# jchristopherson/nonlin

Hardware: AMD Instinct MI355X
Metric: LM iterations/sec on m=4096,n=256 fp64; FD-Jacobian GB/s vs HBM peak (higher is better)
Workload: dtype f64

## Files before the change

nonlin_amd/csrc/nlh_common.h:

```cpp
#pragma once
#include <hip/hip_runtime.h>
#include <stdint.h>
#include <type_traits>

#define NLH_WAVE 64

enum NlhStage : int32_t {
    ST_NEED_JAC = 0,
    ST_HAVE_JAC = 1,
    ST_NE_READY = 2,
    ST_NEED_QR = 3,
    ST_QR_READY = 4,
    ST_TRIAL_READY = 5,
    ST_TRIAL_DONE = 6,
    ST_DONE = 7,
    ST_NEED_PCHOL = 8
};

struct LmState {
    double fnorm, fnorm1, par, delta, xnorm, gnorm, pnorm;
    double temp1n;
    double tailsq;
    int32_t iter, neval, njac;
    int32_t stage;
// ... 394 lines not shown
            for (int h = 0; h < 2; ++h) {
                const double av = a[u + h];
                const bool gt = av > prev;
                const double t = (gt ? prev : av) / (gt ? av : prev), tsq = t * t;
                const double d = (prev == 0.0) ? 0.0 : tsq;
                if (gt && prev != 0.0 && tsq != 1.0) newmax |= 1u << (u + h);
                dd[h] = d;
                prev = fmax(prev, av);
            }
            ddst[u >> 1] = make_double2(dd[0], dd[1]);
        }
        tflags[tid] = (int)newmax;
        __syncthreads();
        if (wid == cw) {
            const int nl = (cl + EL - 1) / EL;
            double d[EL];
            const double2 *mine = reinterpret_cast<const double2 *>(dsv + lane * (EL + 2));
#pragma unroll
            for (int u = 0; u < EL / 2; ++u) { const double2 v2 = mine[u]; d[2 * u] = v2.x; d[2 * u + 1] = v2.y; }
            unsigned long long nm = 0;
#pragma unroll
            for (int k = 0; k < TPR; ++k) nm |= (unsigned long long)(unsigned)tflags[lane * TPR + k] << (k * E);
            const unsigned long long mask = __ballot(nm == 0);
            double t = carry[1];
            const int ntrip = (nl + 7) >> 3;
#pragma unroll 1
            for (int g = 0; g < ntrip; ++g) {
                const unsigned m8 = (unsigned)(mask >> (8 * g)) & 0xffu;
                if (m8 == 0xffu) {
#pragma unroll
                    for (int q = 0; q < 8; ++q) {
                        t = nlh_wave_shr1(t);
#pragma unroll
                        for (int u = 0; u < EL; ++u) t = t + d[u];
                    }
                } else {
#pragma unroll 1
                    for (int q = 0; q < 8; ++q) {
                        t = nlh_wave_shr1(t);
                        if ((m8 >> q) & 1u) {
#pragma unroll
                            for (int u = 0; u < EL; ++u) t = t + d[u];
                        } else if (REGGEN) {
#pragma unroll
                            for (int u = 0; u < EL; ++u) {
                                t = t * (((nm >> u) & 1ull) ? d[u] : 1.0);
                                t = t + d[u];
                            }
                        } else {
                            const int l = 8 * g + q;
                            const unsigned long long nml = ((unsigned long long)(unsigned)__builtin_amdgcn_readlane((int)(nm >> 32), l) << 32)
                                                           | (unsigned)__builtin_amdgcn_readlane((int)nm, l);
#pragma unroll
                            for (int qd = 0; qd < EL; qd += 16) {
                                if (((nml >> qd) & 0xffffull) == 0) {
#pragma unroll
                                    for (int u = qd; u < qd + 16; ++u) t = t + d[u];
                                } else {
#pragma unroll
                                    for (int u = qd; u < qd + 16; ++u) {
                                        t = t * (((nml >> u) & 1ull) ? d[u] : 1.0);
                                        t = t + d[u];
                                    }
                                }
                            }
                        }
                    }
                }
            }
            const int lo = __builtin_amdgcn_readlane(__double2loint(t), 8 * ntrip - 1);
            const int hi = __builtin_amdgcn_readlane(__double2hiint(t), 8 * ntrip - 1);
            double mx = mx_in;
#pragma unroll
            for (int w = 0; w < nw; ++w) mx = fmax(mx, wmax[w]);
            if (lane == 0) { carry[1] = __hiloint2double(hi, lo); carry[0] = mx; }
        }
    }
    __syncthreads();
    const double r = carry[0] * sqrt(1.0 + carry[1]);
    __syncthreads();
    return r;
}

__device__ __forceinline__ void nlh_lds_barrier() { asm volatile("s_waitcnt lgkmcnt(0)\n\ts_barrier" ::: "memory"); }

__device__ __forceinline__ bool nlh_odd_ulps(double c, double inv2ulp)
{
    const double z = c * inv2ulp;
    return z != floor(z);
}
template <int EL>
__device__ __forceinline__ double ordered_possum_wave_int(const double (&d)[EL], double s0, bool &ok)
{
    const long long sb = __double_as_longlong(s0);
    const long long es = sb >> 52;
    const double ulp = __longlong_as_double((es - 52) << 52), hu = 0.5 * ulp, inv2ulp = 0.5 / ulp;
    const double C = __longlong_as_double((es << 52) | (1ll << 51)), lim = 0.25 * __longlong_as_double(es << 52);
    double c0 = 0.0, c1 = 0.0;
    bool fine = true;
#pragma unroll
    for (int u = 0; u < EL; ++u) {
        const double x = d[u];
        fine = fine && (x <= lim);
        const double t = C + x, q = t - C, r = x - q;
        const bool tie = fabs(r) == hu;
        if (__builtin_expect(__builtin_amdgcn_ballot_w64(tie) != 0ull, 0)) {
            const double f = x - hu;
            const double a0 = tie ? f + (nlh_odd_ulps(c0 + f, inv2ulp) ? ulp : 0.0) : q;
            const double a1 = tie ? f + (nlh_odd_ulps(c1 + f, inv2ulp) ? 0.0 : ulp) : q;
            c0 = c0 + a0;
            c1 = c1 + a1;
        } else {
            c0 = c0 + q;
            c1 = c1 + q;
        }
    }
#pragma unroll
    for (int off = 1; off < 64; off <<= 1) {
        const double r0 = __shfl_down(c0, off, 64), r1 = __shfl_down(c1, off, 64);
        const double n0 = c0 + (nlh_odd_ulps(c0, inv2ulp) ? r1 : r0);
        const double n1 = c1 + (nlh_odd_ulps(c1, inv2ulp) ? r0 : r1);
        c0 = n0; c1 = n1;
    }
    const double totl = (sb & 1ll) ? c1 : c0;
    const double tot = __hiloint2double(__builtin_amdgcn_readfirstlane(__double2hiint(totl)), __builtin_amdgcn_readfirstlane(__double2loint(totl)));
    const double out = s0 + tot;
    ok = (__builtin_amdgcn_ballot_w64(!fine) == 0ull) && ((__double_as_longlong(out) >> 52) == es);
    return out;
}

template <int EL, int BSZ, typename Get>
__device__ double norm2_flang_block_lanes_pipe(Get get, int len, double *cd, double *aux, double *wm)
{
    constexpr int CAP = 64 * EL, PADCAP = CAP + 128, E = CAP / BSZ, TPR = EL / E, nw = BSZ / 64;
    static_assert(CAP % BSZ == 0 && EL % E == 0 && E % 2 == 0, "chunk must split evenly");
    const int tid = threadIdx.x, lane = tid & 63, wid = tid >> 6;
    const bool prep = wid < nw, chain = (wid == nw);
    const int nch = (len + CAP - 1) / CAP, i0 = tid * E;
    int *tflags = reinterpret_cast<int *>(aux + 8);
    auto loadabs = [&](int c, double (&a)[E]) __attribute__((always_inline)) {
        const int base = c * CAP, cl = min(CAP, len - base);
#pragma unroll
        for (int u = 0; u < E; ++u) a[u] = (i0 + u < cl) ? fabs(get(base + i0 + u)) : 0.0;
    };
    auto scanmax = [&](int c, const double (&a)[E]) __attribute__((always_inline)) {
        double lm = 0.0;
#pragma unroll
        for (int u = 0; u < E; ++u) lm = fmax(lm, a[u]);
        double sc = lm;
#pragma unroll
        for (int off = 1; off < 64; off <<= 1) {
            const double o = __shfl_up(sc, off, 64);
            if (lane >= off) sc = fmax(sc, o);
        }
        double ex = __shfl_up(sc, 1, 64);
        if (lane == 0) ex = 0.0;
        if (lane == 63) wm[c * nw + wid] = sc;
        return ex;
    };
    double a0[E], a1[E], ex0 = 0.0;
    __syncthreads();
    if (prep) {
        loadabs(0, a0);
        if (nch > 1) loadabs(1, a1);
        ex0 = scanmax(0, a0);
    }
// ... 288 lines not shown
```

nonlin_amd/csrc/nlh_qrx.hip:

```cpp
#include "nlh_qrx.h"
#include "nlh_common.h"
#include "../../include/nonlin_hip.h"
#include <type_traits>
#include <cstdio>
#include <cstdlib>
#include <algorithm>

#ifndef QRX_C
#define QRX_C 10
#endif
#define QRX_TR 64
#define QRX_PAD_ROWS 160
#ifndef QRX_AUX_LOAD
#define QRX_AUX_LOAD 0
#endif
#ifndef QRX_AUX_STORE
#define QRX_AUX_STORE 1
#endif
#ifndef QRX_UF
#define QRX_UF(flush) 16
#endif

typedef unsigned int qrx_u32x2 __attribute__((ext_vector_type(2)));
typedef unsigned int qrx_u32x4 __attribute__((ext_vector_type(4)));
// ... 105 lines not shown

__global__ void __launch_bounds__(256)
k_qrx_init_norms(int m, int n, int ld, int coff, size_t tst, const double *__restrict__ T, QrxWs w, LmVecs v,
                 const LmState *__restrict__ st)
{
    __shared__ __attribute__((aligned(16))) double cd[64 * 64 + 128];
    __shared__ __attribute__((aligned(16))) double aux[40 + 128];
    const int p = w.plist ? w.plist[blockIdx.y] : (int)blockIdx.y, k = blockIdx.x;
    if (p < 0 || (st && st[p].stage != ST_NEED_QR)) return;
    const double *a = T + (size_t)p * tst;
    const double nr = norm2_flang_block_lanes<64, 256>([&](int i) { return a[qrx_at(i, coff + k, ld)]; }, m, cd, aux);
    if (threadIdx.x == 0) {
        v.acnorm[(size_t)p * n + k] = nr;
        w.rdiag[(size_t)p * n + k] = nr;
        w.wa[(size_t)p * n + k] = nr;
        v.ipvt[(size_t)p * n + k] = k;
    }
}

template <bool NORMS>
__global__ void __launch_bounds__(256)
k_qrx_init(int m, int n, int ld, int coff, size_t tst, double *__restrict__ T, const double *__restrict__ fall, QrxWs w, LmVecs v,
           const LmState *__restrict__ st)
{
    const int p = blockIdx.x;
    if (st && st[p].stage != ST_NEED_QR) return;
    const int tid = threadIdx.x, BS = blockDim.x;
    double *a = T + (size_t)p * tst;
    const double *f = fall + (size_t)p * m;
    for (int i = tid; i < m; i += BS) a[qrx_at(i, coff + n, ld)] = f[i];
    for (int k = tid; NORMS && k < n; k += BS) {
        double mx = 0.0, sq = 0.0;
        auto step = [&](double vv) {
            const double av = fabs(vv);
            if (mx == 0.0) {
                mx = av;
            } else if (av > mx) {
                const double t = mx / av, tsq = t * t;
                sq = sq * tsq;
                sq = sq + tsq;
                mx = av;
            } else if (av != 0.0) {
                const double t = av / mx;
                sq = sq + t * t;
            }
        };
        const int nblk = (m + 7) >> 3;
        const double *colp = a + (size_t)(coff + k) * 8;
        double xa[8], xb[8];
        auto ld8 = [&](double (&x)[8], int b) {
#pragma unroll
            for (int r = 0; r < 8; ++r) x[r] = colp[(size_t)b * ld * 8 + r];
        };
        ld8(xa, 0);
        for (int b = 0; b < nblk; b += 2) {
            if (b + 1 < nblk) ld8(xb, b + 1);
#pragma unroll
            for (int r = 0; r < 8; ++r) if (b * 8 + r < m) step(xa[r]);
            if (b + 2 < nblk) ld8(xa, b + 2);
            if (b + 1 < nblk) {
#pragma unroll
                for (int r = 0; r < 8; ++r) if ((b + 1) * 8 + r < m) step(xb[r]);
            }
        }
        const double nr = mx * sqrt(1.0 + sq);
        v.acnorm[(size_t)p * n + k] = nr;
        w.rdiag[(size_t)p * n + k] = nr;
        w.wa[(size_t)p * n + k] = nr;
        v.ipvt[(size_t)p * n + k] = k;
    }
    for (int k = tid; k <= n; k += BS) w.src[(size_t)p * (n + 1) + k] = coff + k;
    for (int c = tid; c < ld; c += BS) w.slotof[(size_t)p * ld + c] = c >= coff ? c - coff : -1;
}

#define QRX_LONG_EL 48
#define QRX_LONG_THREADS 256
#ifndef QRX_LONG_GU
#define QRX_LONG_GU 8
#endif
#ifndef QRX_LONG_SU
#define QRX_LONG_SU 4
#endif
#ifndef QRX_PIV64_WG
#define QRX_PIV64_WG 1
#endif
#define QRX_LONG_MAXCH 96
template <int QRX_NL, bool LONG = false, bool FEW = false>
__global__ void __launch_bounds__(LONG ? QRX_LONG_THREADS : 256, (QRX_NL == 32 && !FEW) ? 4 : (QRX_NL == 64 && !FEW && !LONG) ? QRX_PIV64_WG : 1)
k_qrx_pivot(int p0, int m, int n, int ld, int coff, size_t tst, size_t vst, int j, int cur, int np, int flush, double *__restrict__ T, QrxWs w,
            double *__restrict__ Rall, LmVecs v, const LmState *__restrict__ st)
{
    __shared__ __attribute__((aligned(16))) double cd[LONG ? 2 * (64 * QRX_LONG_EL + 128) : (64 * QRX_NL + (FEW ? 256 : 128))];
    __shared__ __attribute__((aligned(16))) double aux[LONG ? 8 + 256 : 40 + 128];
    __shared__ double wmx[LONG ? 3 * QRX_LONG_MAXCH : 1];
    __shared__ double red[64];
    const int p = p0 + blockIdx.x;
    if (st && st[p].stage != ST_NEED_QR) return;
    const int tid = threadIdx.x, BS = blockDim.x, ldp = n + 1;
#ifdef QRX_DBG_CLK
    long long clk[6]; clk[0] = wall_clock64();
#endif
    int *redi = reinterpret_cast<int *>(red + 32);
    double *rdiag = w.rdiag + (size_t)p * n, *wa = w.wa + (size_t)p * n;
    int32_t *src = w.src + (size_t)p * ldp;
    int32_t *ipvt = v.ipvt + (size_t)p * n;
    double *tpc = w.tp + ((size_t)p * 2 + cur) * QRX_C * ldp;
    double *R = Rall + (size_t)p * n * n;

    const bool onecand = (n - j <= BS);
    int32_t *slotof = w.slotof + (size_t)p * ld;
    const bool fresh = (flush & 2) != 0;
    if (fresh) {
        for (int c = tid; c < ld; c += BS) slotof[c] = (c - coff >= j && c - coff <= n) ? c - coff : -1;
        for (int k = j + tid; k <= n; k += BS) src[k] = coff + k;
    }
    double bv = 0.0, my_tk[QRX_C - 1];
    int bk = 0x7fffffff, my_src = 0, my_ipvt = 0;
    if (onecand) {
        const int k = j + tid;
        if (k < n) {
            bv = rdiag[k]; bk = k;
            my_src = fresh ? coff + k : src[k]; my_ipvt = ipvt[k];
#pragma unroll
            for (int q = 0; q < QRX_C - 1; ++q) my_tk[q] = (q < np) ? tpc[(size_t)q * ldp + k] : 0.0;
        }
    } else {
        for (int k = j + tid; k < n; k += BS) {
            const double d = rdiag[k];
            if (bk == 0x7fffffff || d > bv) { bv = d; bk = k; }
        }
    }
    double rd_j = 0.0, wa_j = 0.0;
    int src_j = 0, ipvt_j = 0, src_0 = 0;
    if (tid == 0) { rd_j = rdiag[j]; wa_j = wa[j]; src_j = fresh ? coff + j : src[j]; ipvt_j = ipvt[j]; src_0 = src[0]; }
    __shared__ uint32_t amx[3 * 16];
    const int kmax = (QRX_NL == 32 && onecand) ? j + block_argmax_first_norms(bv, bk != 0x7fffffff, amx) : block_argmax_first(bv, bk, red, redi);
    double *pub = red + 40;
    int *pubi = reinterpret_cast<int *>(pub + QRX_C);
    if (onecand) {
        if (j + tid == kmax) {
#pragma unroll
            for (int q = 0; q < QRX_C - 1; ++q) pub[q] = my_tk[q];
            pubi[0] = my_src; pubi[1] = my_ipvt;
        }
    } else if (tid == 0) {
        pubi[0] = fresh ? coff + kmax : src[kmax]; pubi[1] = ipvt[kmax];
    } else if (tid <= np) {
        pub[tid - 1] = tpc[(size_t)(tid - 1) * ldp + kmax];
    }
    __syncthreads();
    const int srck = pubi[0];
#ifdef QRX_DBG_CLK
    clk[1] = wall_clock64();
#endif
    double tk[QRX_C];
#pragma unroll
    for (int q = 0; q < QRX_C; ++q) tk[q] = (q < QRX_C - 1 && q < np) ? pub[q] : 0.0;
    if (kmax != j) {
        if (tid == 0) {
            rdiag[kmax] = rd_j;
            wa[kmax] = wa_j;
            ipvt[j] = pubi[1]; ipvt[kmax] = ipvt_j;
            if (j == 0) {
                slotof[src_0] = -1;
                slotof[srck] = kmax;
            } else {
                src[kmax] = src_j;
                slotof[src_j] = kmax;
                slotof[srck] = -1;
            }
        }
        if (tid < np) tpc[(size_t)tid * ldp + kmax] = tpc[(size_t)tid * ldp + j];
        for (int i = tid; i < j; i += BS) {
            const double t = R[(size_t)j * n + i];
            R[(size_t)j * n + i] = R[(size_t)kmax * n + i];
            R[(size_t)kmax * n + i] = t;
        }
    } else if (tid == 0) {
        slotof[srck] = -1;
    }
    const bool move0 = (j == 0 && kmax != 0);
    if (LONG && (flush & 8)) {
        if (tid == 0) {
            QrxStep s;
            s.ajnorm = 0.0; s.ajj = 0.0; s.kmax = kmax; s.srck = srck; s.t0 = np ? tk[0] : 0.0;
            w.step[p] = s;
        }
        return;
    }
    const int src0 = coff;
    const double *__restrict__ Vc = w.V + ((size_t)p * 2 + cur) * QRX_C * vst;
    double *__restrict__ Vn = (flush & 1) ? w.V + ((size_t)p * 2 + (cur ^ 1)) * QRX_C * vst
                                    : w.V + (((size_t)p * 2 + cur) * QRX_C + np) * vst;
    double *Tp = T + (size_t)p * tst;
    const bool staged = !LONG && (m - j <= 64 * QRX_NL);
    double *stage = cd;
    auto spos = [](int i) __attribute__((always_inline)) { return FEW ? i + i / (64 * QRX_NL / 256) : i; };
    constexpr int KEEP = 64 * QRX_NL / 256;
    double keep[KEEP];
#pragma unroll
    for (int u = 0; u < KEEP; ++u) keep[u] = 0.0;
    auto gather4 = [&](int i0, double (&e)[4]) __attribute__((always_inline)) {
        double vq[4][QRX_C - 1], mv[4];
#pragma unroll
        for (int u = 0; u < 4; ++u) {
            const int row = min(i0 + u * BS, m - 1);
            e[u] = Tp[qrx_at(row, srck, ld)];
            mv[u] = move0 ? Tp[qrx_at(row, src0, ld)] : 0.0;
#pragma unroll
            for (int q = 0; q < QRX_C - 1; ++q) vq[u][q] = (q < np) ? Vc[(size_t)q * vst + row] : 0.0;
        }
#pragma unroll
        for (int u = 0; u < 4; ++u) {
#pragma unroll
            for (int q = 0; q < QRX_C - 1; ++q)
                if (q < np) e[u] = e[u] - tk[q] * vq[u][q];
            if (move0 && i0 + u * BS < m) Tp[qrx_at(i0 + u * BS, srck, ld)] = mv[u];
        }
    };
    if (FEW && staged && np == 1 && !move0) {
        double e[KEEP], pv[KEEP];
#pragma unroll
        for (int u = 0; u < KEEP; ++u) {
            const int row = min(j + tid + u * BS, m - 1);
            e[u] = Tp[qrx_at(row, srck, ld)];
            pv[u] = Vc[row];
        }
#pragma unroll
        for (int u = 0; u < KEEP; ++u) { asm volatile("" : "+v"(e[u])); asm volatile("" : "+v"(pv[u])); }
#pragma unroll
        for (int u = 0; u < KEEP; ++u) {
            e[u] = e[u] - tk[0] * pv[u];
            keep[u] = e[u];
            if (j + tid + u * BS < m) stage[spos(tid + u * BS)] = e[u];
        }
    } else if (staged) {
#pragma unroll
        for (int it = 0; it < KEEP / 4; ++it) {
            const int i0 = j + tid + it * 4 * BS;
            if (i0 < m) {
                double e[4];
                gather4(i0, e);
#pragma unroll
                for (int u = 0; u < 4; ++u) {
                    keep[it * 4 + u] = e[u];
                    if (i0 + u * BS < m) stage[spos(i0 + u * BS - j)] = e[u];
                }
            }
        }
    } else if (LONG && np <= 1 && !move0) {
        const int jb = j & ~7, npair = (m - jb + 1) >> 1;
        const double *colp = Tp + qrx_at(jb, srck, ld);
        const size_t blk = (size_t)ld * 8;
        const double t0 = np ? tk[0] : 0.0;
        constexpr int GU = QRX_LONG_GU;
        for (int pb = tid; pb < npair; pb += GU * BS) {
            double2 ax[GU], px[GU];
#pragma unroll
            for (int u = 0; u < GU; ++u) {
                const int pr = min(pb + u * BS, npair - 1);
                ax[u] = *reinterpret_cast<const double2 *>(colp + (size_t)(pr >> 2) * blk + 2 * (pr & 3));
                px[u] = np ? *reinterpret_cast<const double2 *>(Vc + jb + 2 * pr) : make_double2(0.0, 0.0);
            }
#pragma unroll
            for (int u = 0; u < GU; ++u) {
                const int pr = pb + u * BS, row = jb + 2 * pr;
                if (pr >= npair) continue;
                if (np) { ax[u].x = ax[u].x - t0 * px[u].x; ax[u].y = ax[u].y - t0 * px[u].y; }
                if (row >= j && row + 1 < m) *reinterpret_cast<double2 *>(Vn + row) = ax[u];
                else {
                    if (row >= j && row < m) Vn[row] = ax[u].x;
                    if (row + 1 >= j && row + 1 < m) Vn[row + 1] = ax[u].y;
                }
            }
        }
    } else {
        for (int i0 = j + tid; i0 < m; i0 += 4 * BS) {
            double e[4];
            gather4(i0, e);
#pragma unroll
            for (int u = 0; u < 4; ++u)
                if (i0 + u * BS < m) Vn[i0 + u * BS] = e[u];
        }
    }
    __syncthreads();
    const double ejj = staged ? stage[0] : Vn[j];
#ifdef QRX_DBG_CLK
    clk[2] = wall_clock64();
#endif
    double ajnorm;
    if constexpr (LONG) ajnorm = norm2_flang_block_lanes_pipe<QRX_LONG_EL, 192>([&](int i) { return Vn[j + i]; }, m - j, cd, aux, wmx);
    else ajnorm = staged ? norm2_flang_block_lanes<QRX_NL, 256, FEW>([&](int i) { return stage[spos(i)]; }, m - j, cd, aux)
                         : norm2_flang_block_lanes<QRX_NL, 256, FEW>([&](int i) { return Vn[j + i]; }, m - j, cd, aux);
#ifdef QRX_DBG_CLK
    clk[3] = wall_clock64();
#endif
    double ajj = 0.0;
    if (staged) {
        if (ajnorm != 0.0 && ejj < 0.0) ajnorm = -ajnorm;
        const double dn = (ajnorm != 0.0) ? ajnorm : 1.0;
#pragma unroll
        for (int u = 0; u < KEEP; ++u) keep[u] = keep[u] / dn;
#pragma unroll
        for (int u = 0; u < KEEP; ++u) {
            const int i = j + tid + u * BS;
            double t = keep[u];
            if (ajnorm != 0.0 && i == j) { t = t + 1.0; ajj = t; }
            if (i < m) Vn[i] = t;
        }
    } else if (LONG && (flush & 4) && ajnorm != 0.0) {
        if (ejj < 0.0) ajnorm = -ajnorm;
        if (tid == 0) { ajj = ejj / ajnorm + 1.0; Vn[j] = ajj; }
    } else if (LONG && ajnorm != 0.0) {
        if (ejj < 0.0) ajnorm = -ajnorm;
        const int jb = j & ~7, nsec = (m - jb + 7) >> 3;
        for (int sb = tid; sb < nsec; sb += QRX_LONG_SU * BS) {
            double2 tx[QRX_LONG_SU][4];
#pragma unroll
            for (int q = 0; q < QRX_LONG_SU; ++q) {
                const double2 *sp = reinterpret_cast<const double2 *>(Vn + jb + (size_t)min(sb + q * BS, nsec - 1) * 8);
#pragma unroll
                for (int h = 0; h < 4; ++h) tx[q][h] = sp[h];
            }
#pragma unroll
            for (int q = 0; q < QRX_LONG_SU; ++q) {
                const int sc = sb + q * BS, row = jb + sc * 8;
                if (sc >= nsec) continue;
#pragma unroll
                for (int h = 0; h < 4; ++h) {
                    tx[q][h].x = tx[q][h].x / ajnorm;
                    tx[q][h].y = tx[q][h].y / ajnorm;
                    if (row + 2 * h == j) { tx[q][h].x = tx[q][h].x + 1.0; ajj = tx[q][h].x; }
                    if (row + 2 * h + 1 == j) { tx[q][h].y = tx[q][h].y + 1.0; ajj = tx[q][h].y; }
                }
                if (row >= j && row + 8 <= m) {
                    double2 *dp = reinterpret_cast<double2 *>(Vn + row);
#pragma unroll
                    for (int h = 0; h < 4; ++h) dp[h] = tx[q][h];
                } else {
#pragma unroll
                    for (int h = 0; h < 4; ++h) {
                        if (row + 2 * h >= j && row + 2 * h < m) Vn[row + 2 * h] = tx[q][h].x;
                        if (row + 2 * h + 1 >= j && row + 2 * h + 1 < m) Vn[row + 2 * h + 1] = tx[q][h].y;
                    }
                }
            }
        }
    } else if (ajnorm != 0.0) {
        if (ejj < 0.0) ajnorm = -ajnorm;
        for (int i0 = j + tid; i0 < m; i0 += 8 * BS) {
            double t[8];
#pragma unroll
            for (int u = 0; u < 8; ++u) t[u] = Vn[min(i0 + u * BS, m - 1)];
#pragma unroll
            for (int u = 0; u < 8; ++u) {
                t[u] = t[u] / ajnorm;
                if (i0 + u * BS == j) { t[u] = t[u] + 1.0; ajj = t[u]; }
                if (i0 + u * BS < m) Vn[i0 + u * BS] = t[u];
            }
        }
    }
#ifdef QRX_DBG_CLK
    clk[4] = wall_clock64();
    if (tid == 0 && j == 100) printf("pivot j=100: head %lld gather %lld norm %lld scale %lld (x10 ns)\n", clk[1]-clk[0], clk[2]-clk[1], clk[3]-clk[2], clk[4]-clk[3]);
#endif
    if (tid == 0) {
        QrxStep s;
        s.ajnorm = ajnorm; s.ajj = ajj; s.kmax = kmax; s.srck = srck; s.t0 = 0.0;
        w.step[p] = s;
        rdiag[j] = -ajnorm;
    }
}

__global__ void __launch_bounds__(256)
k_qrx_gather_long(int m, int ld, size_t tst, size_t vst, int j, int cur, int np, int flush, const double *__restrict__ T, QrxWs w,
                  const LmState *__restrict__ st)
{
    const int p = blockIdx.y;
    if (st && st[p].stage != ST_NEED_QR) return;
    const QrxStep step = w.step[p];
    const double *Tp = T + (size_t)p * tst;
// ... 1164 lines not shown
        else if (np > QRX_RPW_MAXNP && wide()) f = NLH_QRX_PASS_FOUR_WAVE;
        if (f == NLH_QRX_PASS_WAVE && k.share && nwin >= 2 && nwin <= QRX_SHARE_MAXWIN) f = NLH_QRX_PASS_WAVE_SHARED;
        s.pass = f;
        s.gwin = f == NLH_QRX_PASS_WIDE_HALF ? nhalf : nwin;
        s.lds = wide() ? (int)qrx_rpw_lds(16) : 0;
        s.lds_max = wide() ? s.lds : 65536;
    }

    int next(nlh_qrx_plan_step &s)
    {
        if (j >= n) return 0;
        s.j = j; s.cur = cur; s.tcur = tcur; s.oop = 0;
        s.pivot = pivot_form();
        if (head.sweep == NLH_QRX_SWEEP_COLUMN) {
            s.np = s.flush = s.pf = j > 0;
            s.lo = 0;
            s.pass = NLH_QRX_PASS_COLUMN; s.gwin = n - j;
            s.lds = (int)qrx_col_lds(m, j); s.lds_max = (int)QRX_COL_LDS_MAX;
            np = 1;
        } else {
            s.np = np; s.lo = lo;
            pass_form(s);
            s.pf = (s.flush ? 1 : 0) | (prev_flushed ? 2 : 0);
            const bool wide = s.pass == NLH_QRX_PASS_WIDE || s.pass == NLH_QRX_PASS_WIDE_HALF;
            if (!(s.flush ? qrx_can_flush(np) : np <= QRX_C - 2) || (wide && np > QRX_RPW_MAXNP) || (s.pass == NLH_QRX_PASS_FOUR_WAVE && np >= 8))
                return qrx_plan_bug(s);
            prev_flushed = s.flush;
            s.oop = s.flush && oop_ok && (s.pass == NLH_QRX_PASS_WAVE || s.pass == NLH_QRX_PASS_WAVE_SHARED);
            if (s.oop) tcur ^= 1;
            if (s.flush) { np = 1; lo = j + 1; } else np += 1;
        }
        if (s.flush) cur ^= 1;
        ++j;
        return 1;
    }
};

extern "C" int32_t nlh_qrx_plan(int32_t nprob, int32_t m, int32_t n, int32_t nact, int32_t have_stages, nlh_qrx_plan_head *head,
                                nlh_qrx_plan_step *steps, int32_t cap)
{
    if (nprob < 1 || n < 1 || m < n) return -NLH_INVALID_INPUT_ERROR;
    QrxPlanner plan(nprob, m, n, nact, have_stages != 0, qrx_knobs(), qrx_oop_mode() != 0);
    if (head) *head = plan.head;
    nlh_qrx_plan_step s;
    int more;
    while ((more = plan.next(s)) > 0)
        if (steps && s.j < cap) steps[s.j] = s;
    return more < 0 ? -NLH_INVALID_OPERATION_ERROR : n;
}

bool qrx_wants_second_matrix(int nprob, int m, int n, int nact, bool have_stages)
{
    if (qrx_oop_mode() == 0) return false;
    QrxPlanner plan(nprob, m, n, nact, have_stages, qrx_knobs(), true);
    nlh_qrx_plan_step s;
    while (plan.next(s) > 0)
        if (s.oop) return true;
    return false;
}

struct QrxLaunch {
    hipStream_t stream;
    int nprob, m, n, ld, coff;
    size_t tst, vst;
    double *T[2], *R;
    LmVecs v;
    const LmState *st;
    QrxWs w;
};

static bool launch_pivot(const QrxLaunch &a, const nlh_qrx_plan_step &s)
{
    auto pivot = [&](auto kernel, int threads, int pf) {
        hipLaunchKernelGGL(kernel, dim3(a.nprob), dim3(threads), 0, a.stream, 0, a.m, a.n, a.ld, a.coff, a.tst, a.vst, s.j, s.cur, s.np, pf, a.T[s.tcur], a.w, a.R, a.v, a.st);
    };
    auto scale = [&] {
        hipLaunchKernelGGL(k_qrx_scale_long, dim3((unsigned)(((a.m - s.j) / 2 + 1023) / 1024 + 1), a.nprob), dim3(256), 0, a.stream, a.m, a.vst, s.j, s.cur, s.np,
                           s.pf, a.w, a.st);
    };
    switch (s.pivot) {
    case NLH_QRX_PIVOT_FEW32: pivot(k_qrx_pivot<32, false, true>, 256, s.pf); return true;
    case NLH_QRX_PIVOT_BATCH32: pivot(k_qrx_pivot<32>, 256, s.pf); return true;
    case NLH_QRX_PIVOT_FEW64: pivot(k_qrx_pivot<64, false, true>, 256, s.pf); return true;
    case NLH_QRX_PIVOT_BATCH64: pivot(k_qrx_pivot<64>, 256, s.pf); return true;
    case NLH_QRX_PIVOT_LONG: pivot(k_qrx_pivot<64, true>, QRX_LONG_THREADS, s.pf); return true;
    case NLH_QRX_PIVOT_LONG_SCALED:
        pivot(k_qrx_pivot<64, true>, QRX_LONG_THREADS, s.pf | 4);
        scale();
        return true;
    case NLH_QRX_PIVOT_LONG_SPLIT:
        pivot(k_qrx_pivot<64, true>, QRX_LONG_THREADS, s.pf | 4 | 8);
        hipLaunchKernelGGL(k_qrx_gather_long, dim3((unsigned)(((a.m - (s.j & ~7)) / 2 + 1023) / 1024 + 1), a.nprob), dim3(256), 0, a.stream, a.m, a.ld, a.tst,
                           a.vst, s.j, s.cur, s.np, s.pf, a.T[s.tcur], a.w, a.st);
        hipLaunchKernelGGL(k_qrx_norm_long, dim3(a.nprob), dim3(QRX_NORM_THREADS), 0, a.stream, a.m, a.n, a.vst, s.j, s.cur, s.np, s.pf, a.w, a.st);
        scale();
        return true;
    }
    return false;
}

template <int NP, bool FLUSH>
static bool launch_pass(const QrxLaunch &a, const nlh_qrx_plan_step &s)
{
    const int npl = a.w.plist ? a.w.ny : a.nprob;
    auto pass = [&](auto kernel, int nprob, unsigned grid, int threads, auto... list) {
        hipLaunchKernelGGL(kernel, dim3(grid), dim3(threads), (size_t)s.lds, a.stream, 0, nprob, s.gwin, s.lo, a.m, a.n, a.ld, a.coff, a.tst, a.vst, s.j, s.cur,
                           a.T[s.tcur], a.w.V, a.w.tp, a.w.src, a.w.slotof, a.w.rdiag, a.w.wa, a.w.step, a.R, a.v.qtf, a.st, list...);
    };
    auto lane = [&](auto kernel, unsigned grid, int threads) {
        hipLaunchKernelGGL(kernel, dim3(grid), dim3(threads), (size_t)s.lds, a.stream, 0, a.nprob, s.gwin, s.lo, a.m, a.n, a.ld, a.coff, a.tst, a.vst, s.j,
                           s.cur, a.T[s.tcur], a.T[s.tcur ^ s.oop], a.w.V, a.w.tp, a.w.src, a.w.slotof, a.w.rdiag, a.w.wa, a.w.step, a.R, a.v.qtf, a.st);
    };
    auto tiles = [&](int nprob) { return (unsigned)(((nprob + 7) / 8) * 8 * s.gwin); };
    switch (s.pass) {
    case NLH_QRX_PASS_WIDE:
        if constexpr (NP <= QRX_RPW_MAXNP) { pass(k_qrx_pass_rpw<NP, FLUSH, 16>, npl, tiles(npl), 64 * 16, a.w.plist); return true; }
        break;
    case NLH_QRX_PASS_WIDE_HALF:
        if constexpr (NP <= QRX_RPW_MAXNP) { pass(k_qrx_pass_rpw<NP, FLUSH, 16, 32>, npl, tiles(npl), 64 * 16, a.w.plist); return true; }
        break;
    case NLH_QRX_PASS_FOUR_WAVE:
        if constexpr (NP < 8) { pass(k_qrx_pass_rp<NP, FLUSH, 4>, npl, tiles(npl), 64 * 4, a.w.plist); return true; }
        break;
    case NLH_QRX_PASS_WAVE: lane(k_qrx_pass<NP, FLUSH, false>, tiles(a.nprob), 64); return true;
    case NLH_QRX_PASS_WAVE_SHARED: lane(k_qrx_pass<NP, FLUSH, true>, (unsigned)a.nprob, 64 * s.gwin); return true;
    }
    return false;
}

template <int NP = 0>
static bool dispatch_pass(const QrxLaunch &a, const nlh_qrx_plan_step &s)
{
    if (s.np == NP) {
        if constexpr (qrx_can_flush(NP)) if (s.flush) return launch_pass<NP, true>(a, s);
        if constexpr (NP < QRX_C - 1) if (!s.flush) return launch_pass<NP, false>(a, s);
        return false;
    }
    if constexpr (NP < QRX_C - 1) return dispatch_pass<NP + 1>(a, s);
    return false;
}

static bool launch_pass(const QrxLaunch &a, const nlh_qrx_plan_step &s)
{
    if (s.pass != NLH_QRX_PASS_COLUMN) return dispatch_pass(a, s);
    auto col = [&](auto kernel) {
        hipLaunchKernelGGL(kernel, dim3(s.gwin, a.w.ny), dim3(256), (size_t)s.lds, a.stream, a.m, a.n, a.ld, a.tst, a.vst, s.j, s.cur, a.T[s.tcur], a.w.V, a.w.tp,
                           a.w.src, a.w.rdiag, a.w.wa, a.w.step, a.R, a.v.qtf, a.st, a.w.plist);
    };
    if (s.np) col(k_qrx_pass_col<true>); else col(k_qrx_pass_col<false>);
    return true;
}

template <int NP>
static void qrx_rpw_attr()
{
    const int lim = (int)qrx_rpw_lds(16);
    hipFuncSetAttribute((const void *)k_qrx_pass_rpw<NP, false, 16>, hipFuncAttributeMaxDynamicSharedMemorySize, lim);
    hipFuncSetAttribute((const void *)k_qrx_pass_rpw<NP, false, 16, 32>, hipFuncAttributeMaxDynamicSharedMemorySize, lim);
    if constexpr (qrx_can_flush(NP)) {
        hipFuncSetAttribute((const void *)k_qrx_pass_rpw<NP, true, 16>, hipFuncAttributeMaxDynamicSharedMemorySize, lim);
        hipFuncSetAttribute((const void *)k_qrx_pass_rpw<NP, true, 16, 32>, hipFuncAttributeMaxDynamicSharedMemorySize, lim);
    }
    if constexpr (NP < QRX_RPW_MAXNP) qrx_rpw_attr<NP + 1>();
}

void qrx_init_device()
{
// ... 51 lines not shown
```

Before: 3813.

## Add register-lean norm path for batch 64-lane pivot kernel, raise occupancy

Adds a new blockwise scaled 2-norm routine that processes 32 elements per lane and chains up to two waves. The batch 4096-row pivot kernel uses it and drops the per-thread keep[] array in favour of normalizing through padded LDS. The kernel is split into a step-0 variant and one without it, uniform values are moved to scalar registers, and the launch-bounds occupancy hint goes from 1 to 4 workgroups. The aim is lower register pressure and more waves in flight, at the cost of extra LDS traffic and barriers, and a risk of register spills under the tighter bound.

```diff
diff --git a/nonlin_amd/csrc/nlh_common.h b/nonlin_amd/csrc/nlh_common.h
--- a/nonlin_amd/csrc/nlh_common.h
+++ b/nonlin_amd/csrc/nlh_common.h
@@ -500,6 +500,151 @@
     return r;
 }
 
+__device__ __forceinline__ double nlh_chain_lanes32(const double (&d)[32], unsigned nm, double t, int nl)
+{
+    const unsigned long long mask = __ballot(nm == 0);
+    const int ntrip = (nl + 7) >> 3;
+#pragma unroll 1
+    for (int g = 0; g < ntrip; ++g) {
+        const unsigned m8 = (unsigned)(mask >> (8 * g)) & 0xffu;
+        if (m8 == 0xffu) {
+#pragma unroll
+            for (int q = 0; q < 8; ++q) {
+                t = nlh_wave_shr1(t);
+#pragma unroll
+                for (int u = 0; u < 32; ++u) t = t + d[u];
+            }
+        } else {
+#pragma unroll 1
+            for (int q = 0; q < 8; ++q) {
+                t = nlh_wave_shr1(t);
+                if ((m8 >> q) & 1u) {
+#pragma unroll
+                    for (int u = 0; u < 32; ++u) t = t + d[u];
+                } else {
+                    const unsigned nml = (unsigned)__builtin_amdgcn_readlane((int)nm, 8 * g + q);
+#pragma unroll
+                    for (int qd = 0; qd < 32; qd += 16) {
+                        if (((nml >> qd) & 0xffffu) == 0) {
+#pragma unroll
+                            for (int u = qd; u < qd + 16; ++u) t = t + d[u];
+                        } else {
+#pragma unroll
+                            for (int u = qd; u < qd + 16; ++u) {
+                                t = t * (((nml >> u) & 1u) ? d[u] : 1.0);
+                                t = t + d[u];
+                            }
+                        }
+                    }
+                }
+            }
+        }
+    }
+    const int lo = __builtin_amdgcn_readlane(__double2loint(t), 8 * ntrip - 1);
+    const int hi = __builtin_amdgcn_readlane(__double2hiint(t), 8 * ntrip - 1);
+    return __hiloint2double(hi, lo);
+}
+
+__device__ __forceinline__ void norm2_lanes2_begin(double *aux)
+{
+    __syncthreads();
+    if (threadIdx.x == 0) { aux[32] = 0.0; aux[33] = 0.0; }
+}
+__device__ __forceinline__ void norm2_lanes2_chunk(const double (&x)[16], int cl, double *cd, double *aux)
+{
+    constexpr int EL = 32, E = 16, TPR = EL / E, nw = 4;
+    const int tid = threadIdx.x, lane = tid & 63, wid = tid >> 6;
+    const int cw = nlh_chain_wave(nw), cw2 = (cw + 1) & (nw - 1);
+    double *dsv = cd, *wmax = aux, *carry = aux + 32;
+    int *tflags = reinterpret_cast<int *>(aux + 40);
+    const int i0 = tid * E;
+    double lm = 0.0;
+#pragma unroll
+    for (int u = 0; u < E; ++u) lm = fmax(lm, fabs(x[u]));
+    double sc = lm;
+#pragma unroll
+    for (int off = 1; off < 64; off <<= 1) {
+        const double o = __shfl_up(sc, off, 64);
+        if (lane >= off) sc = fmax(sc, o);
+    }
+    double ex = __shfl_up(sc, 1, 64);
+    if (lane == 0) ex = 0.0;
+    __syncthreads();
+    if (lane == 63) wmax[wid] = sc;
+    __syncthreads();
+    const double mx_in = carry[0];
+    double prev = fmax(mx_in, ex);
+    for (int w = 0; w < wid; ++w) prev = fmax(prev, wmax[w]);
+    unsigned newmax = 0;
+    double2 *ddst = reinterpret_cast<double2 *>(dsv + i0 + 2 * (i0 / EL));
+#pragma unroll
+    for (int u = 0; u < E; u += 2) {
+        double dd[2];
+#pragma unroll
+        for (int h = 0; h < 2; ++h) {
+            const double av = fabs(x[u + h]);
+            const bool gt = av > prev;
+            const double t = (gt ? prev : av) / (gt ? av : prev), tsq = t * t;
+            const double d = (prev == 0.0) ? 0.0 : tsq;
+            if (gt && prev != 0.0 && tsq != 1.0) newmax |= 1u << (u + h);
+            dd[h] = d;
+            prev = fmax(prev, av);
+        }
+        ddst[u >> 1] = make_double2(dd[0], dd[1]);
+    }
+    tflags[tid] = (int)newmax;
+    __syncthreads();
+    const int nl = (cl + EL - 1) / EL;
+    const bool two = nl > 64;
+    const bool first = (wid == cw), second = two && (wid == cw2);
+    double d[EL];
+    unsigned nm = 0;
+    if (first || second) {
+        const int run = (first ? 0 : 64) + lane;
+        const double2 *mine = reinterpret_cast<const double2 *>(dsv + run * (EL + 2));
+#pragma unroll
+        for (int u = 0; u < EL / 2; ++u) { const double2 v2 = mine[u]; d[2 * u] = v2.x; d[2 * u + 1] = v2.y; }
+#pragma unroll
+        for (int k = 0; k < TPR; ++k) nm |= (unsigned)tflags[run * TPR + k] << (k * E);
+    }
+    if (first) {
+        const double s = nlh_chain_lanes32(d, nm, carry[1], min(nl, 64));
+        double mx = mx_in;
+#pragma unroll
+        for (int w = 0; w < nw; ++w) mx = fmax(mx, wmax[w]);
+        if (lane == 0) { carry[1] = s; carry[0] = mx; }
+    }
+    if (two) {
+        __syncthreads();
+        if (second) {
+            const double s = nlh_chain_lanes32(d, nm, carry[1], nl - 64);
+            if (lane == 0) carry[1] = s;
+        }
+    }
+}
+__device__ __forceinline__ double norm2_lanes2_result(const double *aux)
+{
+    __syncthreads();
+    const double r = aux[32] * sqrt(1.0 + aux[33]);
+    __syncthreads();
+    return r;
+}
+
+template <typename Get>
+__device__ double norm2_flang_block_lanes2(Get get, int len, double *cd, double *aux)
+{
+    constexpr int CAP = 128 * 32, E = 16;
+    norm2_lanes2_begin(aux);
+    for (int base = 0; base < len; base += CAP) {
+        const int cl = min(CAP, len - base), i0 = threadIdx.x * E;
+        double x[E];
+#pragma unroll
+        for (int u = 0; u < E; ++u) x[u] = (i0 + u < cl) ? get(base + i0 + u) : 0.0;
+        norm2_lanes2_chunk(x, cl, cd, aux);
+    }
+    return norm2_lanes2_result(aux);
+}
+
 __device__ __forceinline__ void nlh_lds_barrier() { asm volatile("s_waitcnt lgkmcnt(0)\n\ts_barrier" ::: "memory"); }
 
 __device__ __forceinline__ bool nlh_odd_ulps(double c, double inv2ulp)
diff --git a/nonlin_amd/csrc/nlh_qrx.hip b/nonlin_amd/csrc/nlh_qrx.hip
--- a/nonlin_amd/csrc/nlh_qrx.hip
+++ b/nonlin_amd/csrc/nlh_qrx.hip
@@ -211,15 +211,17 @@
 #define QRX_LONG_SU 4
 #endif
 #ifndef QRX_PIV64_WG
-#define QRX_PIV64_WG 1
+#define QRX_PIV64_WG 4
 #endif
 #define QRX_LONG_MAXCH 96
-template <int QRX_NL, bool LONG = false, bool FEW = false>
+template <int QRX_NL, bool LONG = false, bool FEW = false, bool STEP0 = true>
 __global__ void __launch_bounds__(LONG ? QRX_LONG_THREADS : 256, (QRX_NL == 32 && !FEW) ? 4 : (QRX_NL == 64 && !FEW && !LONG) ? QRX_PIV64_WG : 1)
 k_qrx_pivot(int p0, int m, int n, int ld, int coff, size_t tst, size_t vst, int j, int cur, int np, int flush, double *__restrict__ T, QrxWs w,
             double *__restrict__ Rall, LmVecs v, const LmState *__restrict__ st)
 {
-    __shared__ __attribute__((aligned(16))) double cd[LONG ? 2 * (64 * QRX_LONG_EL + 128) : (64 * QRX_NL + (FEW ? 256 : 128))];
+    constexpr bool B64 = (QRX_NL == 64 && !LONG && !FEW);
+    static_assert(STEP0 || B64, "only the batch instance of the 4096-row kernel has a form without step 0");
+    __shared__ __attribute__((aligned(16))) double cd[LONG ? 2 * (64 * QRX_LONG_EL + 128) : (64 * QRX_NL + (B64 ? 512 : FEW ? 256 : 128))];
     __shared__ __attribute__((aligned(16))) double aux[LONG ? 8 + 256 : 40 + 128];
     __shared__ double wmx[LONG ? 3 * QRX_LONG_MAXCH : 1];
     __shared__ double red[64];
@@ -278,13 +280,16 @@
         pub[tid - 1] = tpc[(size_t)(tid - 1) * ldp + kmax];
     }
     __syncthreads();
-    const int srck = pubi[0];
+    const int srck = B64 ? __builtin_amdgcn_readfirstlane(pubi[0]) : pubi[0];
 #ifdef QRX_DBG_CLK
     clk[1] = wall_clock64();
 #endif
     double tk[QRX_C];
 #pragma unroll
-    for (int q = 0; q < QRX_C; ++q) tk[q] = (q < QRX_C - 1 && q < np) ? pub[q] : 0.0;
+    for (int q = 0; q < QRX_C; ++q) {
+        tk[q] = (q < QRX_C - 1 && q < np) ? pub[q] : 0.0;
+        if (B64) tk[q] = __hiloint2double(__builtin_amdgcn_readfirstlane(__double2hiint(tk[q])), __builtin_amdgcn_readfirstlane(__double2loint(tk[q])));
+    }
     if (kmax != j) {
         if (tid == 0) {
             rdiag[kmax] = rd_j;
@@ -308,7 +313,7 @@
     } else if (tid == 0) {
         slotof[srck] = -1;
     }
-    const bool move0 = (j == 0 && kmax != 0);
+    const bool move0 = STEP0 && (j == 0 && kmax != 0);
     if (LONG && (flush & 8)) {
         if (tid == 0) {
             QrxStep s;
@@ -324,7 +329,7 @@
     double *Tp = T + (size_t)p * tst;
     const bool staged = !LONG && (m - j <= 64 * QRX_NL);
     double *stage = cd;
-    auto spos = [](int i) __attribute__((always_inline)) { return FEW ? i + i / (64 * QRX_NL / 256) : i; };
+    auto spos = [](int i) __attribute__((always_inline)) { return B64 ? i + 2 * (i / 16) : FEW ? i + i / (64 * QRX_NL / 256) : i; };
     constexpr int KEEP = 64 * QRX_NL / 256;
     double keep[KEEP];
 #pragma unroll
@@ -372,7 +377,7 @@
                 gather4(i0, e);
 #pragma unroll
                 for (int u = 0; u < 4; ++u) {
-                    keep[it * 4 + u] = e[u];
+                    if (!B64) keep[it * 4 + u] = e[u];
                     if (i0 + u * BS < m) stage[spos(i0 + u * BS - j)] = e[u];
                 }
             }
@@ -413,19 +418,59 @@
         }
     }
     __syncthreads();
-    const double ejj = staged ? stage[0] : Vn[j];
+    double ejj = 0.0;
+    if constexpr (B64) { if (tid == 0) aux[34] = staged ? stage[0] : Vn[j]; }
+    else ejj = staged ? stage[0] : Vn[j];
 #ifdef QRX_DBG_CLK
     clk[2] = wall_clock64();
 #endif
-    double ajnorm;
+    double ajnorm, ajj0 = 0.0;
     if constexpr (LONG) ajnorm = norm2_flang_block_lanes_pipe<QRX_LONG_EL, 192>([&](int i) { return Vn[j + i]; }, m - j, cd, aux, wmx);
+    else if constexpr (B64) {
+        if (staged) {
+            const int cl = m - j, e0 = tid * 16;
+            double x[16];
+            const double2 *sp = reinterpret_cast<const double2 *>(stage + spos(e0));
+#pragma unroll
+            for (int u = 0; u < 8; ++u) {
+                const double2 v2 = sp[u];
+                x[2 * u] = (e0 + 2 * u < cl) ? v2.x : 0.0;
+                x[2 * u + 1] = (e0 + 2 * u + 1 < cl) ? v2.y : 0.0;
+            }
+            norm2_lanes2_begin(aux);
+            norm2_lanes2_chunk(x, cl, cd, aux);
+            ajnorm = norm2_lanes2_result(aux);
+            ejj = aux[34];
+#ifdef QRX_DBG_CLK
+            clk[3] = wall_clock64();
+#endif
+            if (ajnorm != 0.0 && ejj < 0.0) ajnorm = -ajnorm;
+            const double dn = (ajnorm != 0.0) ? ajnorm : 1.0;
+#pragma unroll
+            for (int u = 0; u < 16; ++u) x[u] = x[u] / dn;
+            if (ajnorm != 0.0 && tid == 0) { x[0] = x[0] + 1.0; ajj0 = x[0]; }
+            double2 *dp = reinterpret_cast<double2 *>(stage + spos(e0));
+#pragma unroll
+            for (int u = 0; u < 8; ++u) dp[u] = make_double2(x[2 * u], x[2 * u + 1]);
+            __syncthreads();
+#pragma unroll
+            for (int u = 0; u < 16; ++u) {
+                const int i = tid + u * BS;
+                if (i < cl) Vn[j + i] = stage[spos(i)];
+            }
+        } else {
+            ajnorm = norm2_flang_block_lanes2([&](int i) { return Vn[j + i]; }, m - j, cd, aux);
+            ejj = aux[34];
+        }
+    }
     else ajnorm = staged ? norm2_flang_block_lanes<QRX_NL, 256, FEW>([&](int i) { return stage[spos(i)]; }, m - j, cd, aux)
                          : norm2_flang_block_lanes<QRX_NL, 256, FEW>([&](int i) { return Vn[j + i]; }, m - j, cd, aux);
 #ifdef QRX_DBG_CLK
-    clk[3] = wall_clock64();
-#endif
-    double ajj = 0.0;
-    if (staged) {
+    if (!(B64 && staged)) clk[3] = wall_clock64();
+#endif
+    double ajj = ajj0;
+    if (B64 && staged) {
+    } else if (staged) {
         if (ajnorm != 0.0 && ejj < 0.0) ajnorm = -ajnorm;
         const double dn = (ajnorm != 0.0) ? ajnorm : 1.0;
 #pragma unroll
@@ -1756,7 +1801,10 @@
     case NLH_QRX_PIVOT_FEW32: pivot(k_qrx_pivot<32, false, true>, 256, s.pf); return true;
     case NLH_QRX_PIVOT_BATCH32: pivot(k_qrx_pivot<32>, 256, s.pf); return true;
     case NLH_QRX_PIVOT_FEW64: pivot(k_qrx_pivot<64, false, true>, 256, s.pf); return true;
-    case NLH_QRX_PIVOT_BATCH64: pivot(k_qrx_pivot<64>, 256, s.pf); return true;
+    case NLH_QRX_PIVOT_BATCH64:
+        if (s.j == 0) pivot(k_qrx_pivot<64, false, false, true>, 256, s.pf);
+        else pivot(k_qrx_pivot<64, false, false, false>, 256, s.pf);
+        return true;
     case NLH_QRX_PIVOT_LONG: pivot(k_qrx_pivot<64, true>, QRX_LONG_THREADS, s.pf); return true;
     case NLH_QRX_PIVOT_LONG_SCALED:
         pivot(k_qrx_pivot<64, true>, QRX_LONG_THREADS, s.pf | 4);
```

New measurement: 3863, median of 6. 1.01x the previous value.
